# audexdev/Lossless-Audio-Codec

Hardware: AMD Instinct MI355X
Metric: encode Msamples/s at 1/2/4/8 MI355X; byte-identical .lac vs CPU ref (higher is better)
Workload: dtype int64

## Files before the change

### lossless-audio-codec_amd/csrc/api_core.cpp

```cpp
#include "encoder_impl.h"

namespace lacx_host {

Knobs read_knobs() {
    Knobs k;
    auto set = [](const char* name) {
        const char* v = std::getenv(name);
        return v != nullptr;
    };
    auto num = [](const char* name) -> unsigned long long {
        const char* v = std::getenv(name);
        return v ? std::strtoull(v, nullptr, 0) : 0ull;
    };
    k.stream_priority = !set("LACX_NO_STREAM_PRIORITY");
    if (const char* v = std::getenv("LACX_FUSED_EMIT")) k.fused_emit = *v != '0';
    k.direct_packer = set("LACX_DIRECT_PACKER");
    k.packer = !set("LACX_NO_PACKER");
    k.persistent = !set("LACX_NO_PERSISTENT");
    k.debug_drain = set("LACX_DEBUG_DRAIN");
    k.two_copy_streams = !set("LACX_ONE_COPY_STREAM");
    if (const char* v = std::getenv("LACX_STREAM_PRIO")) {
        int a = 0, b = 0, c = 0;
        if (std::sscanf(v, "%d,%d,%d", &a, &b, &c) == 3) {
            k.prio_main = a;
            k.prio_chunks = b;
            k.prio_pack = c;
        }
    }
    k.front_halves = !set("LACX_NO_FRONT_HALVES");
    k.tune.fold_front = !set("LACX_NO_FRONT_FOLD");
    k.lazy_repair = !set("LACX_NO_LAZY_REPAIR");
    k.silent_template = !set("LACX_NO_SILENT_TEMPLATE");
    k.pinned_cap_bytes = num("LACX_PINNED_CAP_BYTES");
    k.debug_skip = (uint32_t)num("LACX_DEBUG_SKIP");
    k.pipe_chunks = (uint32_t)num("LACX_PIPE_CHUNKS");
    if (const char* v = std::getenv("LACX_PIPE_SPLIT")) k.pipe_split = v;
    k.drain_fence = (uint32_t)num("LACX_DRAIN_FENCE");
    if (const char* v = std::getenv("LACX_FANOUT_EXCHANGE")) k.fanout_exchange = std::strcmp(v, "host") == 0 ? 1u : (std::strcmp(v, "rccl") == 0 ? 2u : 0u);
    k.tune.persistent_grid = (uint32_t)num("LACX_PERSISTENT_GRID");
    k.tune.pack_nap = (int)num("LACX_PACK_NAP");
    k.tune.pack_grid = (int)num("LACX_PACK_GRID");
    k.tune.no_pairs = set("LACX_NO_PAIRS");
    return k;
}

double ms_since(clk::time_point t0) { return std::chrono::duration<double, std::milli>(clk::now() - t0).count(); }

int fail(lacx_encoder* e, int code, const std::string& msg) {
    if (e) e->err = msg;
    return code;
}

int hip_fail(lacx_encoder* e, hipError_t err, const char* what) {
    return fail(e, LACX_E_DEVICE, std::string(what) + ": " + hipGetErrorString(err));
}

void big_copy(uint8_t* dst, const uint8_t* src, uint64_t n) {
    constexpr uint64_t kPiece = 4ull << 20;
    const unsigned hw = std::thread::hardware_concurrency();
    const uint64_t want = std::min<uint64_t>(std::min<uint64_t>(8, hw ? hw : 1), n / kPiece);
    if (want < 2) {
        std::memcpy(dst, src, n);
        return;
    }
    std::vector<std::thread> pool;
    const uint64_t per = (n / want + 4095) & ~4095ull;
    for (uint64_t t = 1; t < want; ++t) {
        const uint64_t o = t * per;
        if (o >= n) break;
        pool.emplace_back([=] { std::memcpy(dst + o, src + o, std::min(per, n - o)); });
    }
    std::memcpy(dst, src, std::min(per, n));
    for (auto& th : pool) th.join();
}

int ensure_device(lacx_encoder* e) {
    if (e->device_ready) return LACX_OK;
    int count = 0;
    const hipError_t ce = hipGetDeviceCount(&count);
    if (ce != hipSuccess || count <= 0)
        return fail(e, LACX_E_DEVICE, "no HIP device available: the LAC analysis path has no CPU fallback");
    int dev = e->cfg.device;
    if (dev < 0) HIP_TRY(e, hipGetDevice(&dev), "hipGetDevice");
    if (dev >= count) return fail(e, LACX_E_DEVICE, "HIP device ordinal out of range");
    HIP_TRY(e, hipSetDevice(dev), "hipSetDevice");
    e->device = dev;
    int least = 0, greatest = 0;
    (void)hipDeviceGetStreamPriorityRange(&least, &greatest);
    const bool prio = e->knobs.stream_priority && greatest < least;
    const int normal = (greatest + least) / 2 > greatest ? (greatest + least) / 2 : std::min(greatest + 1, least);
    auto level = [&](int code) { return code < 0 ? greatest : (code == 0 ? normal : least); };
    int i = 0;
    for (auto& s : e->stream) {
        if (prio) {
            const int p = level(i == 0 ? e->knobs.prio_main : (i == kStreams - 1 ? 0 : e->knobs.prio_chunks));
            HIP_TRY(e, hipStreamCreateWithPriority(&s, hipStreamNonBlocking, p), "hipStreamCreate");
        } else {
            HIP_TRY(e, hipStreamCreateWithFlags(&s, hipStreamNonBlocking), "hipStreamCreate");
        }
        ++i;
    }
    for (auto& row : e->ev)
        for (auto& ev : row) HIP_TRY(e, hipEventCreate(&ev), "hipEventCreate");
    for (auto& ev : e->done) HIP_TRY(e, hipEventCreateWithFlags(&ev, hipEventDisableTiming), "hipEventCreate");
    for (auto& ev : e->copied) HIP_TRY(e, hipEventCreateWithFlags(&ev, hipEventDisableTiming), "hipEventCreate");
    HIP_TRY(e, hipEventCreateWithFlags(&e->prologue, hipEventDisableTiming), "hipEventCreate");
    for (auto& ev : e->aux_ev) HIP_TRY(e, hipEventCreateWithFlags(&ev, hipEventDisableTiming), "hipEventCreate");
    HIP_TRY(e, hipHostMalloc((void**)&e->h_totals, sizeof(unsigned long long) * kMaxChunks, 0), "hipHostMalloc");
    HIP_TRY(e, hipHostMalloc((void**)&e->h_err, sizeof(uint32_t) * (kMaxChunks + 8), 0), "hipHostMalloc");
    HIP_TRY(e, hipStreamCreateWithPriority(&e->pack_stream, hipStreamNonBlocking, level(e->knobs.prio_pack)), "hipStreamCreate");
    HIP_TRY(e, hipEventCreateWithFlags(&e->pack_done, hipEventDisableTiming), "hipEventCreate");
    HIP_TRY(e, hipStreamCreateWithFlags(&e->copy_stream, hipStreamNonBlocking), "hipStreamCreate");
    HIP_TRY(e, hipStreamCreateWithFlags(&e->copy_stream2, hipStreamNonBlocking), "hipStreamCreate");
    HIP_TRY(e, hipHostMalloc((void**)&e->h_tspan, sizeof(unsigned long long) * 2 * kMaxChunks, 0), "hipHostMalloc");
    e->device_ready = true;
    return LACX_OK;
}

EmitPool& pool_of(lacx_encoder* e) {
    if (!e->pool) {
        unsigned nt = e->cfg.emit_threads ? e->cfg.emit_threads : std::thread::hardware_concurrency();
        if (nt == 0) nt = 1;
        e->pool.reset(new EmitPool(nt > 1 ? nt - 1 : 0));
    }
    return *e->pool;
}

void free_workspace(lacx_encoder* e) {
    if (e->ws.plans) (void)hipFree(e->ws.plans);
    if (e->ws.bplans) (void)hipFree(e->ws.bplans);
    if (e->ws.need_probe) (void)hipFree(e->ws.need_probe);
    if (e->ws.need_full) (void)hipFree(e->ws.need_full);
    if (e->ws.acorr) (void)hipFree(e->ws.acorr);
    if (e->ws.lpcs) (void)hipFree(e->ws.lpcs);
    if (e->ws.sums) (void)hipFree(e->ws.sums);
    if (e->ws.badidx) (void)hipFree(e->ws.badidx);
    if (e->ws.front_ctr) (void)hipFree(e->ws.front_ctr);
    if (e->ws.block_off) (void)hipFree(e->ws.block_off);
    if (e->ws.table) (void)hipFree(e->ws.table);
    if (e->ws.stream_pre) (void)hipFree(e->ws.stream_pre);
    if (e->zero_region) (void)hipFree(e->zero_region);
    e->zero_region = nullptr;
    e->d_tspan = nullptr;
    e->d_work_ctr = nullptr;
    e->d_silent = nullptr;
    e->ws = DeviceWorkspace{};
    e->ws_blocks = 0;
}

int ensure_workspace(lacx_encoder* e, uint32_t nblocks) {
    if (nblocks > e->ws_blocks) {
        free_workspace(e);
        const size_t slots = (size_t)nblocks * kSlotsPerBlock;
        HIP_TRY(e, hipMalloc((void**)&e->ws.plans, slots * sizeof(ChannelPlan)), "hipMalloc(plans)");
        HIP_TRY(e, hipMalloc((void**)&e->ws.bplans, (size_t)nblocks * sizeof(BlockPlan)), "hipMalloc(bplans)");
        HIP_TRY(e, hipMalloc((void**)&e->ws.need_probe, (size_t)nblocks * 4), "hipMalloc(need)");
        HIP_TRY(e, hipMalloc((void**)&e->ws.need_full, (size_t)nblocks * 4), "hipMalloc(need)");
        HIP_TRY(e, hipMalloc((void**)&e->ws.acorr, slots * 13 * sizeof(int64_t)), "hipMalloc(acorr)");
        HIP_TRY(e, hipMalloc((void**)&e->ws.lpcs, slots * sizeof(LpcSet)), "hipMalloc(lpcs)");
        HIP_TRY(e, hipMalloc((void**)&e->ws.sums, (size_t)nblocks * 12 * sizeof(unsigned long long)), "hipMalloc(sums)");
        HIP_TRY(e, hipMalloc((void**)&e->ws.badidx, (size_t)nblocks * 2 * sizeof(uint32_t)), "hipMalloc(badidx)");
        HIP_TRY(e, hipMalloc((void**)&e->ws.front_ctr, (size_t)nblocks * 2 * sizeof(uint32_t)), "hipMalloc(front counters)");
        HIP_TRY(e, hipMemset(e->ws.front_ctr, 0, (size_t)nblocks * 2 * sizeof(uint32_t)), "hipMemset(front counters)");
        HIP_TRY(e, hipStreamSynchronize(nullptr), "hipStreamSynchronize");
        HIP_TRY(e, hipMalloc((void**)&e->ws.block_off, ((size_t)nblocks + kMaxChunks + 1) * sizeof(unsigned long long)),
                "hipMalloc(block_off)");
        HIP_TRY(e, hipMalloc((void**)&e->ws.table, (size_t)nblocks * 2 * sizeof(uint32_t)), "hipMalloc(table)");
        HIP_TRY(e, hipMalloc((void**)&e->ws.stream_pre, ((size_t)nblocks + 1) * sizeof(unsigned long long)), "hipMalloc(stream prefixes)");

        {
            const size_t items = (size_t)nblocks * 2 + 4;
            const size_t ranges = items / kPackerRangeItems + 2;
            const size_t bytes = items * (2 * sizeof(unsigned long long) + 2 * sizeof(uint32_t)) +
                                 sizeof(unsigned long long) * 2 * kMaxChunks + sizeof(uint32_t) * (kMaxChunks + 8) +
                                 ranges * (sizeof(unsigned long long) + sizeof(uint32_t)) + 16 +
                                 sizeof(uint32_t) * 8 * (kMaxChunks + 1) +
                                 16 + sizeof(SilentTemplate);
            e->zero_bytes = (bytes + 15) & ~(size_t)15;
            HIP_TRY(e, hipMalloc((void**)&e->zero_region, e->zero_bytes), "hipMalloc(zeroed region)");
            uint8_t* p = e->zero_region;
            e->ws.size_rec = reinterpret_cast<unsigned long long*>(p);
            p += items * sizeof(unsigned long long);
            e->ws.ready_rec = reinterpret_cast<unsigned long long*>(p);
            p += items * sizeof(unsigned long long);
            e->d_tspan = reinterpret_cast<unsigned long long*>(p);
            p += sizeof(unsigned long long) * 2 * kMaxChunks;
            e->ws.emitted = reinterpret_cast<uint32_t*>(p);
            p += items * sizeof(uint32_t);
            e->ws.packed = reinterpret_cast<uint32_t*>(p);
            p += items * sizeof(uint32_t);
            e->ws.err_flag = reinterpret_cast<uint32_t*>(p);
            p += sizeof(uint32_t) * (kMaxChunks + 8);
            p = reinterpret_cast<uint8_t*>((reinterpret_cast<uintptr_t>(p) + 7) & ~(uintptr_t)7);
            e->d_range_end = reinterpret_cast<unsigned long long*>(p);
            p += ranges * sizeof(unsigned long long);
            e->d_range_cnt = reinterpret_cast<uint32_t*>(p);
            p += ranges * sizeof(uint32_t);
            p = reinterpret_cast<uint8_t*>((reinterpret_cast<uintptr_t>(p) + 3) & ~(uintptr_t)3);
            e->d_work_ctr = reinterpret_cast<uint32_t*>(p);
            p += sizeof(uint32_t) * 8 * (kMaxChunks + 1);
            p = reinterpret_cast<uint8_t*>((reinterpret_cast<uintptr_t>(p) + 15) & ~(uintptr_t)15);
            e->d_silent = reinterpret_cast<SilentTemplate*>(p);
        }
        e->ws_blocks = nblocks;
    }
    if (nblocks > e->h_blocks) {
        if (e->h_plans) (void)hipHostFree(e->h_plans);
        if (e->h_bplans) (void)hipHostFree(e->h_bplans);
        e->h_plans = nullptr;
        e->h_bplans = nullptr;
        e->h_blocks = 0;
        HIP_TRY(e, hipHostMalloc((void**)&e->h_plans, (size_t)nblocks * kSlotsPerBlock * sizeof(ChannelPlan), 0),
                "hipHostMalloc(plans)");
        HIP_TRY(e, hipHostMalloc((void**)&e->h_bplans, (size_t)nblocks * sizeof(BlockPlan), 0),
                "hipHostMalloc(bplans)");
        e->h_blocks = nblocks;
    }
    return LACX_OK;
}

int ensure_slots(lacx_encoder* e, uint32_t nblocks, int channels, int bit_depth) {
    const unsigned long long stride = (unsigned long long)kMaxBlock * ((bit_depth ? bit_depth : e->cfg.bit_depth) == 16 ? 3u : 5u);
    const unsigned long long need = stride * nblocks * (unsigned)channels + 64u;
    if (const int rc = grow(e, e->slot_mem, need)) return rc;
    e->ws.slots = e->slot_mem.as<uint8_t>();
    e->ws.slot_stride = stride;
    return LACX_OK;
}

int grow(lacx_encoder* e, Buf& b, uint64_t need) {
    const DevErr d = buf_grow(b, need, 0);
    return d ? hip_fail(e, d.e, d.what) : LACX_OK;
}

int ensure_pcm(lacx_encoder* e, uint64_t frames, bool) { return grow(e, e->pcm, frames); }

int validate_stream_args(lacx_encoder* e, const void* left, uint64_t frames) {
    if (left == nullptr || frames == 0) return fail(e, LACX_E_INVALID, "left channel must not be empty");
    if (!rate_ok(e->cfg.sample_rate))
        return fail(e, LACX_E_INVALID, "unsupported sample rate: " + std::to_string(e->cfg.sample_rate));
    if (!(e->cfg.bit_depth == 16 || e->cfg.bit_depth == 24))
        return fail(e, LACX_E_INVALID, "unsupported bit depth: " + std::to_string((int)e->cfg.bit_depth));
    if (e->cfg.stereo_mode > 2)
        return fail(e, LACX_E_INVALID, "unsupported stereo mode: " + std::to_string((int)e->cfg.stereo_mode));
    return LACX_OK;
}

AnalyzeParams make_params(const lacx_encoder* e, uint64_t frames, int channels, int stereo_mode, int bit_depth, int layout) {
    return make_params(param_base(e), frames, channels, stereo_mode, bit_depth, layout);
}

LaunchSet one_stream_set(const AnalyzeParams& prm, const int32_t* left, const int32_t* right, uint32_t fuse_items,
                         uint64_t out_cap) {
    StreamDesc sd{};
    sd.prm = prm;
    sd.left = left;
    sd.right = right;
    sd.first_block = 0;
    sd.first_wg = 0;
    sd.fuse_items = fuse_items;
    sd.out_base = 0;
    sd.out_cap = out_cap;
    return single_set(sd);
}
const LaunchSet& bind(LaunchSet& ls) {
    if (ls.br.table == nullptr) ls.streams = &ls.br.single;
    return ls;
}

DeviceWorkspace ws_at(const DeviceWorkspace& ws, uint32_t first_block) {
    DeviceWorkspace w = ws;
    const size_t s = (size_t)first_block * kSlotsPerBlock;
    w.plans += s;
    w.bplans += first_block;
    w.need_probe += first_block;
    w.need_full += first_block;
    w.acorr += s * 13;
    w.lpcs += s;
    w.sums += (size_t)first_block * 12;
    w.badidx += (size_t)first_block * 2;
    if (w.front_ctr) w.front_ctr += (size_t)first_block * 2;
    w.table += (size_t)first_block * 2;
    return w;
}

void add_chunk_timing(lacx_encoder* e, int c) {
    float f = 0;
    if (hipEventElapsedTime(&f, e->ev[c][0], e->ev[c][4]) == hipSuccess) e->timing.analysis_ms += f;
    if (hipEventElapsedTime(&f, e->ev[c][0], e->ev[c][1]) == hipSuccess) e->timing.ingest_ms += f;
    if (hipEventElapsedTime(&f, e->ev[c][1], e->ev[c][2]) == hipSuccess) e->timing.probe_ms += f;
    if (hipEventElapsedTime(&f, e->ev[c][2], e->ev[c][3]) == hipSuccess) e->timing.full_ms += f;
    (void)hipGetLastError();
}

void count_slots(lacx_encoder* e, uint32_t first, uint32_t count) {
    uint64_t fs = 0, ps = 0;
    for (uint32_t b = first; b < first + count; ++b) {
        const ChannelPlan* s = e->h_plans + (size_t)b * kSlotsPerBlock;
        for (int i = 0; i < 4; ++i) fs += s[i].valid;
        for (int i = 4; i < kSlotsPerBlock; ++i) ps += s[i].valid;
    }
    e->timing.full_slots += fs;
    e->timing.probe_slots += ps;
}

int check_sample_range(lacx_encoder* e, uint32_t nb) {
    e->bad_channel = -1;
    for (int pass = 0; pass < 2; ++pass) {
        for (uint32_t b = 0; b < nb; ++b) {
            const BlockPlan& bp = e->h_bplans[b];
            if (!bp.invalid) continue;
            const bool is_right = (bp.first_bad >> 31) != 0;
            if ((pass == 0) == is_right) continue;
            const uint64_t idx = (uint64_t)b * kMaxBlock + (bp.first_bad & 0x7FFFFFFFu);
            e->bad_channel = is_right ? 1 : 0;
            e->bad_index = idx;
            return fail(e, LACX_E_INVALID,
                        std::string(is_right ? "right" : "left") + " sample at index " + std::to_string(idx) +
                            " is outside the configured PCM bit depth");
        }
    }
    return LACX_OK;
}

void reset_device_timing(lacx_encoder* e) {
    e->timing.analysis_ms = e->timing.ingest_ms = e->timing.probe_ms = e->timing.full_ms = 0;
    e->timing.full_slots = e->timing.probe_slots = 0;
    e->timing.full_launches = 0;
}

StreamParams stream_params(const lacx_config& c, int channels) {
    StreamParams sp;
    sp.sample_rate = c.sample_rate;
    sp.bit_depth = c.bit_depth;
    sp.channels = (uint8_t)channels;
    sp.stereo_mode = channels == 2 ? c.stereo_mode : 0;
    return sp;
// ... 146 lines not shown
```

### lossless-audio-codec_amd/csrc/k_front.hip

```cpp
#include <hip/hip_runtime.h>

#include "kernels_internal.h"
#include "x87.h"

namespace lacx {

__device__ __forceinline__ uint64_t zz64(int64_t v) {
    return v >= 0 ? ((uint64_t)v << 1) : ((((uint64_t)(-(v + 1))) << 1) | 1u);
}

__device__ __forceinline__ uint64_t approx_rice_bits(uint64_t sum, uint64_t count) {
    if (count == 0) return 0;
    const uint64_t mean = (sum + (count >> 1)) / count;
    uint32_t k = mean <= 1u ? 0u : 64u - (uint32_t)__clzll((long long)(mean - 1u));
    k = k > 31u ? 31u : k;
    return (sum >> k) + count * (uint64_t)(k + 1u);
}

constexpr int kIngestTile = 4096;
static_assert(kIngestThreads == kProbe, "one probe sample per thread");

__device__ __forceinline__ bool slot_channel_used(const AnalyzeParams& prm, int ch) {
    if (prm.channels == 1) return ch == 0;
    if (prm.stereo_mode == 0) return ch < 2;
    if (prm.stereo_mode == 1) return ch >= 2;
    return true;
}

__device__ __forceinline__ void reduce13(const int64_t* acc, unsigned long long* s_ac, int64_t* out, int tid) {
    if (tid < 13) s_ac[tid] = 0;
    __syncthreads();
#pragma unroll
    for (int k = 0; k < 13; ++k) {
        const uint64_t t = wave_sum_u64((uint64_t)acc[k]);
        if ((tid & 63) == 0) atomicAdd(&s_ac[k], (unsigned long long)t);
    }
    __syncthreads();
    if (tid < 13) out[tid] = (int64_t)s_ac[tid];
    __syncthreads();
}

__device__ __forceinline__ void stereo_block(const AnalyzeParams& prm, uint32_t blk, uint32_t nb, bool live, int tid,
                                             const unsigned long long* __restrict__ sums, const uint32_t* __restrict__ badidx,
                                             BlockPlan* __restrict__ bplans, uint32_t* __restrict__ need_probe,
                                             uint32_t* __restrict__ need_full);

__device__ __forceinline__ void ingest_done(uint32_t* __restrict__ front_ctr, unsigned int* s_last, const AnalyzeParams& prm,
                                            uint32_t blk, uint32_t nb, const unsigned long long* __restrict__ sums,
                                            const uint32_t* __restrict__ badidx, BlockPlan* __restrict__ bplans,
                                            uint32_t* __restrict__ need_probe, uint32_t* __restrict__ need_full) {
    if (!front_ctr) return;
    const int tid = threadIdx.x;
    if (tid == 0) {
        asm volatile("s_waitcnt vmcnt(0)" ::: "memory");
        *s_last = atomicAdd(&front_ctr[(size_t)blk * 2], 1u) == 3u ? 1u : 0u;
    }
    __syncthreads();
    if (*s_last == 0u || tid >= 64) return;
    if (tid == 0) front_ctr[(size_t)blk * 2] = 0u;
    stereo_block(prm, blk, nb, tid < 16, tid, sums, badidx, bplans, need_probe, need_full);
}

__global__ __launch_bounds__(kIngestThreads, 5) void k_ingest(BatchRef br, unsigned long long* __restrict__ sums,
                                                           uint32_t* __restrict__ badidx,
                                                           int64_t* __restrict__ acorr, uint32_t* __restrict__ front_ctr,
                                                           BlockPlan* __restrict__ bplans, uint32_t* __restrict__ need_probe,
                                                           uint32_t* __restrict__ need_full) {
    __shared__ int4 s_plane[4][kIngestThreads + 1];
    __shared__ __align__(16) int32_t s_win[3][12 + kProbe];
    __shared__ unsigned long long s_ac[13];
    __shared__ unsigned long long s_sum[3];
    __shared__ unsigned int s_bad;
    uint32_t blk, chsel;
    xcd_slot(blockIdx.x, 4u, gridDim.x >> 2, blk, chsel);
    const StreamDesc sd = stream_of_block_uniform(br, blk);
    const AnalyzeParams prm = sd.prm;
    const int32_t* __restrict__ L = sd.left;
    const int32_t* __restrict__ R = sd.right;
    const uint32_t lblk = blk - sd.first_block;
    const int ch = (int)chsel;
    const bool used = slot_channel_used(prm, ch);
    const bool container_bounds = prm.layout == PCM_INTERLEAVED_I16 || (prm.layout == PCM_INTERLEAVED_I24 && prm.bit_depth == 24);
    const bool validate = ch < 2 && ch < prm.channels && prm.bit_depth != 0 && !container_bounds;
    const uint32_t nb = block_frames(prm, lblk);
    if (!used && !validate) {
        if (ch < 2 && threadIdx.x == 0) agent_store(&badidx[blk * 2 + ch], 0xFFFFFFFFu);
        ingest_done(front_ctr, &s_bad, prm, blk, nb, sums, badidx, bplans, need_probe, need_full);
        return;
    }
    const int tid = threadIdx.x, lane = tid & 63;
    const int64_t bstart = (int64_t)lblk * kMaxBlock;
    const SlotSrc src = slot_src(prm, L, R, ch);
    const bool est = prm.channels == 2 && prm.stereo_mode == 2;
    const int32_t lo = prm.bit_depth == 16 ? -32768 : -0x800000;
    const int32_t hi = prm.bit_depth == 16 ? 32767 : 0x7FFFFF;
    if (tid < 3) s_sum[tid] = 0;
    if (tid == 0) s_bad = 0xFFFFFFFFu;
    if (tid < 4) s_plane[tid][0] = make_int4(0, 0, 0, 0);
    __syncthreads();

    constexpr int kPerThread = kIngestTile / kIngestThreads;
    static_assert(kPerThread == 16, "four 4-sample groups per thread and tile");
    int64_t acc[13];
#pragma unroll
    for (int k = 0; k < 13; ++k) acc[k] = 0;
    uint64_t sraw = 0, sdif = 0, sant = 0;
    uint32_t bad = 0xFFFFFFFFu;
    for (uint32_t base = 0; base < nb; base += kIngestTile) {
        const uint32_t first = base + 16u * (uint32_t)tid;
        const int rem = (int)nb - (int)first;
        const int cnt = rem < 0 ? 0 : (rem > 16 ? 16 : rem);
        int32_t w[28];
        load_chunk<16>(src, bstart + first, cnt, bstart + (int64_t)nb - 1, w + 12);
#pragma unroll
        for (int i = 0; i < 16; ++i) {
            if (i >= cnt) w[12 + i] = 0;
            else if (validate && (w[12 + i] < lo || w[12 + i] > hi)) bad = bad < first + (uint32_t)i ? bad : first + (uint32_t)i;
        }
#pragma unroll
        for (int c = 0; c < 4; ++c)
            s_plane[c][tid + 1] = make_int4(w[12 + 4 * c], w[13 + 4 * c], w[14 + 4 * c], w[15 + 4 * c]);
        __syncthreads();
        int4 carry = make_int4(0, 0, 0, 0);
        if (tid >= 1 && tid <= 3) carry = s_plane[tid][kIngestThreads];
#pragma unroll
        for (int c = 1; c < 4; ++c) {
            const int4 h = s_plane[c][tid];
            w[4 * (c - 1)] = h.x;
            w[4 * (c - 1) + 1] = h.y;
            w[4 * (c - 1) + 2] = h.z;
            w[4 * (c - 1) + 3] = h.w;
        }
        if (used) {
#pragma unroll
            for (int i = 0; i < 16; ++i) {
#pragma unroll
                for (int k = 0; k < 13; ++k) acc[k] += (int64_t)w[12 + i] * (int64_t)w[12 + i - k];
            }
            if (est) {
                auto zz32 = [](int32_t v) { return ((uint32_t)v << 1) ^ (uint32_t)(v >> 31); };
                uint32_t traw = 0, tdif = 0, tant = 0;
#pragma unroll
                for (int i = 0; i < 16; ++i) {
                    if (i < cnt) {
                        const int32_t x0 = w[12 + i], prev = w[11 + i];
                        const uint32_t raw = zz32(x0);
                        const bool head = (first + (uint32_t)i) == 0u;
                        traw += raw;
                        tdif += head ? raw : zz32((int32_t)((uint32_t)x0 - (uint32_t)prev));
                        tant += head ? raw : zz32((int32_t)((uint32_t)x0 + (uint32_t)prev));
                    }
                }
                sraw += traw;
                sdif += tdif;
                sant += tant;
            }
        }
        __syncthreads();
        if (tid >= 1 && tid <= 3) s_plane[tid][0] = carry;
    }
    if (used) reduce13(acc, s_ac, acorr + ((size_t)blk * kSlotsPerBlock + ch) * 13, tid);

    if (est && nb > (uint32_t)kFullCompareLimit) {
        if (tid < 36) s_win[tid / 12][tid % 12] = 0;
        for (int w = 1; w <= 3; ++w) {
            const SlotGeom g = slot_geom(prm, lblk, w * 4 + ch);
            s_win[w - 1][12 + tid] = slot_fetch(src, g.start + tid);
        }
        __syncthreads();
        const int wv = tid >> 6;
        if (wv < 3) {
            int32_t v[16];
#pragma unroll
            for (int c = 0; c < 4; ++c) {
                const int4 q = *reinterpret_cast<const int4*>(&s_win[wv][4 * lane + 4 * c]);
                v[4 * c] = q.x;
                v[4 * c + 1] = q.y;
                v[4 * c + 2] = q.z;
                v[4 * c + 3] = q.w;
            }
            int64_t* out = acorr + ((size_t)blk * kSlotsPerBlock + (wv + 1) * 4 + ch) * 13;
#pragma unroll
            for (int k = 0; k < 13; ++k) {
                int64_t a = 0;
#pragma unroll
                for (int i = 0; i < 4; ++i) a += (int64_t)v[12 + i] * (int64_t)v[12 + i - k];
                const uint64_t t = wave_sum_u64((uint64_t)a);
                if (lane == 0) out[k] = (int64_t)t;
            }
        }
    }

    if (est) {
        const uint64_t t0 = wave_sum_u64(sraw), t1 = wave_sum_u64(sdif), t2 = wave_sum_u64(sant);
        if (lane == 0) {
            atomicAdd(&s_sum[0], (unsigned long long)t0);
            atomicAdd(&s_sum[1], (unsigned long long)t1);
            atomicAdd(&s_sum[2], (unsigned long long)t2);
        }
    }
    if (bad != 0xFFFFFFFFu) atomicMin(&s_bad, bad);
    __syncthreads();
    if (tid == 0) {
        if (est) {
            agent_store(&sums[(size_t)blk * 12 + ch], s_sum[0]);
            agent_store(&sums[(size_t)blk * 12 + 4 + ch], s_sum[1]);
            agent_store(&sums[(size_t)blk * 12 + 8 + ch], s_sum[2]);
        }
        if (validate || ch < 2) agent_store(&badidx[blk * 2 + ch], s_bad);
    }
    __syncthreads();
    ingest_done(front_ctr, &s_bad, prm, blk, nb, sums, badidx, bplans, need_probe, need_full);
}

constexpr int kStereoLanes = 16;
__device__ __forceinline__ void stereo_block(const AnalyzeParams& prm, uint32_t blk, uint32_t nb, bool live, int tid,
                                             const unsigned long long* __restrict__ sums, const uint32_t* __restrict__ badidx,
                                             BlockPlan* __restrict__ bplans, uint32_t* __restrict__ need_probe,
                                             uint32_t* __restrict__ need_full) {
    const int sub = tid & (kStereoLanes - 1), grp = tid & ~(kStereoLanes - 1);
    const bool stereo = prm.channels == 2;
    const bool est = stereo && prm.stereo_mode == 2;
    uint64_t bits = 0;
    if (est && live && sub < 12) bits = approx_rice_bits(agent_load(&sums[(size_t)blk * 12 + sub]), nb);
    auto from = [&](int lane_in_group) {
        const uint32_t lo = (uint32_t)__shfl((int)(uint32_t)bits, grp + lane_in_group, 64);
        const uint32_t hi = (uint32_t)__shfl((int)(uint32_t)(bits >> 32), grp + lane_in_group, 64);
        return ((uint64_t)hi << 32) | lo;
    };
    uint64_t chbits[4];
    bool active = false;
#pragma unroll
    for (int c = 0; c < 4; ++c) {
        const uint64_t raw = from(c), dif = from(4 + c), ant = from(8 + c);
        uint64_t mn = raw < dif ? raw : dif;
        if (ant < mn) mn = ant;
        chbits[c] = mn;
        active = active || (raw < dif) || (ant < dif);
    }
    if (!live || sub != 0) return;
    BlockPlan bp;
    bp.choose_ms = 0;
    bp.uncertain = 0;
    bp.est_ms = 0;
    const uint32_t badl = agent_load(&badidx[blk * 2]), badr = stereo ? agent_load(&badidx[blk * 2 + 1]) : 0xFFFFFFFFu;
    bp.invalid = (badl != 0xFFFFFFFFu) || (badr != 0xFFFFFFFFu);
    bp.first_bad = (badl != 0xFFFFFFFFu) ? badl : (badr != 0xFFFFFFFFu ? (badr | 0x80000000u) : 0xFFFFFFFFu);
    bp.frames = nb;
    bp.pad = 0;
    uint32_t nprobe = 0, nfull = 0;
    if (!stereo) {
        nfull = 1u;
    } else if (prm.stereo_mode == 0) {
        nfull = 0x3u;
    } else if (prm.stereo_mode == 1) {
        nfull = 0xCu;
        bp.choose_ms = 1;
    } else {
        const uint64_t lr = chbits[0] + chbits[1], ms = chbits[2] + chbits[3];
        const uint64_t smaller = lr < ms ? lr : ms;
        const uint64_t diff = lr >= ms ? lr - ms : ms - lr;
        bp.est_ms = ms < lr;
        bp.choose_ms = bp.est_ms;
        bp.uncertain = smaller == 0 || diff == 0 || active || diff <= smaller / 100u;
        if (!bp.uncertain) {
            nfull = bp.est_ms ? 0xCu : 0x3u;
        } else if (nb <= (uint32_t)kFullCompareLimit) {
            nfull = 0xFu;
        } else if (agent_load(&sums[(size_t)blk * 12]) == 0ull && agent_load(&sums[(size_t)blk * 12 + 1]) == 0ull) {
            nfull = 0x3u;
            bp.choose_ms = 0;
        } else {
            nprobe = 0xFFF0u;
        }
    }
    bplans[blk] = bp;
    need_probe[blk] = nprobe;
    need_full[blk] = nfull;
}

__global__ __launch_bounds__(64) void k_stereo(BatchRef br, const unsigned long long* __restrict__ sums,
                                               const uint32_t* __restrict__ badidx, BlockPlan* __restrict__ bplans,
                                               uint32_t* __restrict__ need_probe, uint32_t* __restrict__ need_full) {
    const int tid = threadIdx.x;
    const uint32_t blk = blockIdx.x * (64 / kStereoLanes) + (uint32_t)(tid / kStereoLanes);
    const bool live = blk < br.total_blocks;
    const StreamDesc sd = stream_of_block(br, live ? blk : 0u);
    const uint32_t nb = live ? block_frames(sd.prm, blk - sd.first_block) : 0u;
    stereo_block(sd.prm, blk, nb, live, tid, sums, badidx, bplans, need_probe, need_full);
}


__global__ __launch_bounds__(kLevThreads) void k_levinson(BatchRef br, const int64_t* __restrict__ acorr,
                                                          const uint32_t* __restrict__ need_probe,
                                                          LpcSet* __restrict__ lpcs) {
    extern __shared__ __align__(16) unsigned char lev_raw[];
    LevMem& lm = *reinterpret_cast<LevMem*>(lev_raw);
    const uint32_t id = blockIdx.x * kLevThreads + threadIdx.x;
    const uint32_t nblk = br.total_blocks;
    const int slot = (int)(id / nblk);
    const uint32_t blk = id % nblk;
    if (slot >= kSlotsPerBlock) return;
    const StreamDesc sd = stream_of_block(br, blk);
    const AnalyzeParams prm = sd.prm;
    const SlotGeom g = slot_geom(prm, blk - sd.first_block, slot);
    if (!g.defined) return;
    if (prm.channels == 2 && slot < 4) {
        if (prm.stereo_mode == 0 && (slot & 3) >= 2) return;
        if (prm.stereo_mode == 1 && (slot & 3) < 2) return;
    }
    if (slot >= 4 && !((need_probe[blk] >> slot) & 1u)) return;
    const uint32_t gid = blk * kSlotsPerBlock + (uint32_t)slot;
    const int mvo = (g.n > 1) ? (int)((g.n - 1 < 32u) ? g.n - 1 : 32u) : 0;
    struct LdsArray {
        uint64_t (*m)[kLevThreads];
        uint32_t (*es)[kLevThreads];
        int lane;
        __device__ xf80 get(int i) const {
            const uint32_t w = es[i][lane];
            return xf80{m[i][lane], (int32_t)(w & 0x7FFFFFFFu) - (1 << 21), w >> 31};
        }
        __device__ void set(int i, xf80 x) {
            m[i][lane] = x.m;
            es[i][lane] = (x.s << 31) | ((uint32_t)(x.e + (1 << 21)) & 0x7FFFFFFFu);
        }
    };
    const int lane = (int)threadIdx.x;
    LdsArray Rv{lm.m[0], lm.es[0], lane}, av{lm.m[1], lm.es[1], lane}, pv{lm.m[2], lm.es[2], lane};
    const int64_t* r = acorr + (size_t)gid * 13;
    LpcSet* out = &lpcs[gid];
    levinson_candidates_t([r](int i) { return r[i]; }, mvo, Rv, av, pv,
                          [out](int ci, int j, int16_t v) { out->coef[ci][j] = v; },
                          [out](int ci, uint8_t v) { out->used[ci] = v; });
    out->pad = 0;
}

__global__ __launch_bounds__(64) void k_decide(BatchRef br, int phase, BlockPlan* __restrict__ bplans,
                                               const uint32_t* __restrict__ need_probe,
                                               uint32_t* __restrict__ need_full,
                                               const ChannelPlan* __restrict__ plans) {
    const int tid = threadIdx.x, sub = tid & 15;
    const uint32_t blk = blockIdx.x * 4u + (uint32_t)(tid >> 4);
    if (br.table == nullptr && (br.single.prm.channels != 2 || br.single.prm.stereo_mode != 2)) return;
    const bool live = blk < br.total_blocks;
    BlockPlan bp{};
    if (live) bp = bplans[blk];
    const bool mine = live && bp.uncertain &&
                      (phase == 1 ? need_probe[blk] != 0 : bp.frames <= (uint32_t)kFullCompareLimit);
    const bool take = mine && (phase == 1 ? sub >= 4 : sub < 4);
    const uint32_t bytes = take ? plans[(size_t)blk * kSlotsPerBlock + sub].payload_bytes : 0u;
    const bool is_ms = (sub & 3) >= 2;
    uint32_t lr = is_ms ? 0u : bytes, ms = is_ms ? bytes : 0u;
#pragma unroll
    for (int d = 1; d < 16; d <<= 1) {
        lr += (uint32_t)__shfl_xor((int)lr, d, 64);
        ms += (uint32_t)__shfl_xor((int)ms, d, 64);
    }
    if (!mine || sub != 0) return;
    bp.choose_ms = ms < lr;
    bplans[blk] = bp;
    if (phase == 1) need_full[blk] = bp.choose_ms ? 0xCu : 0x3u;
}

hipError_t set_kernel_attrs_front() {
    return hipFuncSetAttribute(reinterpret_cast<const void*>(&k_levinson), hipFuncAttributeMaxDynamicSharedMemorySize,
                               (int)sizeof(LevMem));
}

}
```

### lossless-audio-codec_amd/csrc/lacx_types.h

```cpp
#pragma once
#include <stddef.h>
#include <stdint.h>

struct lacx_block_info;
struct lacx_run_detector;
struct lacx_run;
struct lacx_loudness_row;
struct lacx_truepeak_row;
struct lacx_spectrum_row;

namespace lacx {

constexpr int kMaxBlock = 16384;
constexpr int kMaxParts = 256;
constexpr int kMinPartition = 32;
constexpr int kMaxPartitionOrder = 8;
constexpr size_t kDecodeTailPad = 128;
constexpr int kProbe = 256;
constexpr int kFullCompareLimit = 4096;

enum : int { CH_L = 0, CH_R = 1, CH_M = 2, CH_S = 3 };

constexpr int kSlotsPerBlock = 16;

struct LpcSet {
    int16_t coef[5][13];
    uint8_t used[5];
    uint8_t pad;
};

struct ChannelPlan {
    uint8_t predictor_type;
    uint8_t order;
    uint8_t partition_order;
    uint8_t valid;
    int16_t coef[12];
    uint32_t payload_bytes;
    uint64_t total_bits;
    uint8_t part_mode_k[kMaxParts];
};

struct BlockPlan {
    uint8_t choose_ms;
    uint8_t uncertain;
    uint8_t est_ms;
    uint8_t invalid;
    uint32_t frames;
    uint32_t first_bad;
    uint32_t pad;
};

struct AnalyzeParams {
    uint64_t frames;
    uint32_t num_blocks;
    uint32_t first_block;
    int32_t channels;
    int32_t stereo_mode;
    int32_t bit_depth;
    int32_t zero_run;
    int32_t partitioning;
    uint32_t debug_skip;
    int32_t layout;
    uint32_t stream_base;
};

struct StreamDesc {
    AnalyzeParams prm;
    const int32_t* left;
    const int32_t* right;
    uint32_t first_block;
    uint32_t first_wg;
    uint32_t fuse_items;
    uint32_t pad;
    unsigned long long out_base;
    unsigned long long out_cap;
};

struct BatchRef {
    const StreamDesc* table;
    uint32_t nstreams;
    uint32_t total_blocks;
    StreamDesc single;
};

struct VerifySource {
    const void* data0;
    const void* data1;
    uint32_t layout;
    uint32_t pad;
};
struct VerifyWords {
    unsigned long long count;
    unsigned long long key;
    int32_t decoded, source;
    uint32_t block;
    uint32_t pad;
};

struct DigestWords {
    uint32_t raw;
    uint32_t pad;
};
struct DigestSource {
    const void* data0;
    const void* data1;
    unsigned long long frames;
    uint32_t layout;
    uint8_t channels, bit_depth, pad[2];
};
constexpr unsigned long long kDigestClean = ~0ull;
struct DigestPcmArgs {
    uint32_t nitems = 0;
    unsigned long long total_units = 0;
    const unsigned long long* unit_off = nullptr;
    const DigestSource* src = nullptr;
    DigestWords* res = nullptr;
    unsigned long long* bad = nullptr;
};

struct DecodeItem {
    int32_t* left;
    int32_t* right;
    uint8_t* wav;
    unsigned long long frame0;
    unsigned long long frames;
    unsigned long long pay_off;
    uint32_t block0, blocks;
    uint32_t pay_bits;
    uint8_t channels, stereo_mode, bit_depth, version;
};
struct WindowOut {
    void* left;
    void* right;
    unsigned long long start;
    unsigned long long frames;
};
struct DecodeArgs {
    uint32_t nitems = 0, total_blocks = 0;
    const DecodeItem* items = nullptr;
    const uint32_t* blk_item = nullptr;
    uint32_t lanes = 0;
    const uint32_t* lane_blk = nullptr;
    uint32_t nv2 = 0;
    const uint32_t* v2_items = nullptr;
    const uint8_t* payload = nullptr;
    const unsigned long long* byte_off = nullptr;
    const unsigned long long* frame_off = nullptr;
    uint32_t* status = nullptr;
    uint8_t* ms_flag = nullptr;
    bool wav = false;
    const unsigned long long* unit_off = nullptr;
    unsigned long long total_units = 0;
    const WindowOut* window = nullptr;
    bool f32 = false;
    const VerifySource* verify = nullptr;
    VerifyWords* verify_res = nullptr;
    DigestWords* digest = nullptr;
    const uint32_t* present = nullptr;
    uint32_t* block_raw = nullptr;
    const uint32_t* block_expect = nullptr;
    const uint32_t* judged = nullptr;
    bool no_output = false;
};
struct BlockPcmArgs {
    DigestPcmArgs pcm;
    uint32_t grid = 0;
    const unsigned long long* block_off = nullptr;
    uint32_t* raw = nullptr;
};
struct StatsAcc;
struct StatsArgs {
    DecodeArgs dec;
    StatsAcc* rows = nullptr;
};
struct StatsPcmArgs {
    DigestPcmArgs pcm;
    uint32_t grid = 0;
    const unsigned long long* block_off = nullptr;
    StatsAcc* rows = nullptr;
};
struct RunsItem;
struct RunsList;
struct RunsRow;
struct RunsArgs {
    DecodeArgs dec;
    uint32_t nitems = 0;
    unsigned long long total_tiles = 0;
    const unsigned long long* tile_off = nullptr;
    const RunsItem* items = nullptr;
    const lacx_run_detector* dets = nullptr;
    RunsList* lists = nullptr;
    RunsRow* rows = nullptr;
    lacx_run* runs = nullptr;
    const DigestSource* src = nullptr;
    unsigned long long* bad = nullptr;
};
constexpr uint32_t kInspectPartSlots = 256;
static_assert(kInspectPartSlots == (uint32_t)kMaxParts, "a channel block has at most kMaxParts partitions");
struct InspectArgs {
    DecodeArgs dec;
    lacx_block_info* rows = nullptr;
    uint8_t* mode_k = nullptr;
    uint32_t* part_bits = nullptr;
};
constexpr uint32_t kLoudChunk = 256;
struct LoudFilter {
    double sb[3], sna[2];
    double hb[3], hna[2];
    double A[4][4];
};
struct LoudState {
    double s[4];
};
struct LoudPartial {
    double p[2];
};
struct LoudItem {
    const void* data0;
    const void* data1;
    unsigned long long frames;
    unsigned long long used;
    unsigned long long lane0;
    unsigned long long row0;
    uint32_t chunks, rows;
    uint32_t sub, layout;
    uint8_t channels, bit_depth, rate, validate;
    uint32_t pad;
};
struct LoudArgs {
    uint32_t nitems = 0;
    unsigned long long total_chunks = 0, total_rows = 0;
    const LoudFilter* filters = nullptr;
    const LoudItem* items = nullptr;
    const unsigned long long* chunk_off = nullptr;
    const unsigned long long* row_off = nullptr;
    LoudState* states = nullptr;
    LoudPartial* partials = nullptr;
    lacx_loudness_row* rows = nullptr;
    unsigned long long* bad = nullptr;
};
constexpr uint32_t kTpTileFrames = 1024;
constexpr uint32_t kTpThreads = 256;
constexpr uint32_t kTpTaps = 12, kTpPhases = 4;
constexpr uint32_t kTpFlush = kTpTaps - 1;
constexpr uint32_t kTpHistory = 12;
constexpr uint32_t kTpRowFrames = 16384;
constexpr uint32_t kTpPosBits = 18;
struct TpAcc {
    unsigned long long key[2];
    uint32_t sample_peak[2];
    uint32_t pad[2];
};
struct TpItem {
    const void* data0;
    const void* data1;
    unsigned long long frames;
    unsigned long long row0;
    uint32_t tiles, rows;
    uint32_t layout;
    uint8_t channels, bit_depth, validate, pad;
};
struct TpArgs {
    uint32_t nitems = 0;
    unsigned long long total_tiles = 0, total_rows = 0;
    const TpItem* items = nullptr;
    const unsigned long long* tile_off = nullptr;
    TpAcc* rows = nullptr;
    unsigned long long* bad = nullptr;
};
constexpr uint32_t kSpThreads = 256;
constexpr uint32_t kSpBands = 64;
constexpr uint32_t kSpRowFrames = 16384;
constexpr uint32_t kSpMinLog = 8, kSpMaxLog = 12;
struct SpItem {
    const void* data0;
    const void* data1;
    unsigned long long frames;
    unsigned long long row0;
    unsigned long long windows;
    uint32_t rows;
    uint32_t layout;
    uint8_t channels, bit_depth, validate, pad[5];
};
struct SpArgs {
    uint32_t nitems = 0;
    uint32_t logn = 0;
    unsigned long long total_rows = 0;
    const SpItem* items = nullptr;
    const unsigned long long* row_off = nullptr;
    const double* window = nullptr;
    const double* twiddle = nullptr;
    lacx_spectrum_row* rows = nullptr;
    unsigned long long* bad = nullptr;
};
}
```

Before: 24760.

## Compute ingest autocorrelation with int8 MFMA on split byte planes

Replaces the per-thread int64 VALU autocorrelation loop in k_ingest with int8 MFMA (16x16x64) products. Samples are split into signed byte planes (3 for 16-bit, 4 for 24-bit) and the 13 lags are recombined from the shifted plane products. It also lowers launch bounds occupancy from 5 to 3 workgroups and enlarges the LDS staging buffer. The VALU path stays reachable through a debug bit set by LACX_INGEST_MFMA=0. The risks are exactness of the plane recombination, extra LDS traffic, and lower occupancy.

Result: slower. 24430 (-1.3%).

```diff
diff --git a/lossless-audio-codec_amd/csrc/api_core.cpp b/lossless-audio-codec_amd/csrc/api_core.cpp
--- a/lossless-audio-codec_amd/csrc/api_core.cpp
+++ b/lossless-audio-codec_amd/csrc/api_core.cpp
@@ -33,6 +33,9 @@
     k.silent_template = !set("LACX_NO_SILENT_TEMPLATE");
     k.pinned_cap_bytes = num("LACX_PINNED_CAP_BYTES");
     k.debug_skip = (uint32_t)num("LACX_DEBUG_SKIP");
+    if (const char* v = std::getenv("LACX_INGEST_MFMA")) {
+        if (*v == '0') k.debug_skip |= lacx::kIngestValuBit;
+    }
     k.pipe_chunks = (uint32_t)num("LACX_PIPE_CHUNKS");
     if (const char* v = std::getenv("LACX_PIPE_SPLIT")) k.pipe_split = v;
     k.drain_fence = (uint32_t)num("LACX_DRAIN_FENCE");
diff --git a/lossless-audio-codec_amd/csrc/k_front.hip b/lossless-audio-codec_amd/csrc/k_front.hip
--- a/lossless-audio-codec_amd/csrc/k_front.hip
+++ b/lossless-audio-codec_amd/csrc/k_front.hip
@@ -18,6 +18,9 @@
 }
 
 constexpr int kIngestTile = 4096;
+#ifndef LACX_INGEST_WGS
+#define LACX_INGEST_WGS 3
+#endif
 static_assert(kIngestThreads == kProbe, "one probe sample per thread");
 
 __device__ __forceinline__ bool slot_channel_used(const AnalyzeParams& prm, int ch) {
@@ -61,12 +64,231 @@
     stereo_block(prm, blk, nb, tid < 16, tid, sums, badidx, bplans, need_probe, need_full);
 }
 
-__global__ __launch_bounds__(kIngestThreads, 5) void k_ingest(BatchRef br, unsigned long long* __restrict__ sums,
+struct IngestBlock {
+    SlotSrc src;
+    int64_t bstart;
+    uint32_t nb;
+    int32_t lo, hi;
+    bool validate, used, est;
+    uint64_t sraw, sdif, sant;
+    uint32_t bad;
+};
+
+__device__ __forceinline__ void ingest_check16(IngestBlock& ib, uint32_t first, int cnt, int32_t* x) {
+#pragma unroll
+    for (int i = 0; i < 16; ++i) {
+        if (i >= cnt) x[i] = 0;
+        else if (ib.validate && (x[i] < ib.lo || x[i] > ib.hi)) ib.bad = ib.bad < first + (uint32_t)i ? ib.bad : first + (uint32_t)i;
+    }
+}
+
+__device__ __forceinline__ int ingest_fetch16(IngestBlock& ib, uint32_t first, int32_t* x) {
+    const int rem = (int)ib.nb - (int)first;
+    const int cnt = rem < 0 ? 0 : (rem > 16 ? 16 : rem);
+    load_chunk<16>(ib.src, ib.bstart + first, cnt, ib.bstart + (int64_t)ib.nb - 1, x);
+    ingest_check16(ib, first, cnt, x);
+    return cnt;
+}
+
+__device__ __forceinline__ void ingest_proxy16(IngestBlock& ib, uint32_t first, int cnt, const int32_t* x) {
+    auto zz32 = [](int32_t v) { return ((uint32_t)v << 1) ^ (uint32_t)(v >> 31); };
+    uint32_t traw = 0, tdif = 0, tant = 0;
+#pragma unroll
+    for (int i = 0; i < 16; ++i) {
+        if (i < cnt) {
+            const int32_t x0 = x[i], prev = x[i - 1];
+            const uint32_t raw = zz32(x0);
+            const bool head = (first + (uint32_t)i) == 0u;
+            traw += raw;
+            tdif += head ? raw : zz32((int32_t)((uint32_t)x0 - (uint32_t)prev));
+            tant += head ? raw : zz32((int32_t)((uint32_t)x0 + (uint32_t)prev));
+        }
+    }
+    ib.sraw += traw;
+    ib.sdif += tdif;
+    ib.sant += tant;
+}
+
+__device__ __forceinline__ void ingest_valu(IngestBlock& ib, int4 (*s_plane)[kIngestThreads + 1], unsigned long long* s_ac,
+                                         int64_t* out) {
+    const int tid = threadIdx.x;
+    if (tid < 4) s_plane[tid][0] = make_int4(0, 0, 0, 0);
+    __syncthreads();
+    static_assert(kIngestTile / kIngestThreads == 16, "four 4-sample groups per thread and tile");
+    int64_t acc[13];
+#pragma unroll
+    for (int k = 0; k < 13; ++k) acc[k] = 0;
+    for (uint32_t base = 0; base < ib.nb; base += kIngestTile) {
+        const uint32_t first = base + 16u * (uint32_t)tid;
+        int32_t w[28];
+        const int cnt = ingest_fetch16(ib, first, w + 12);
+#pragma unroll
+        for (int c = 0; c < 4; ++c)
+            s_plane[c][tid + 1] = make_int4(w[12 + 4 * c], w[13 + 4 * c], w[14 + 4 * c], w[15 + 4 * c]);
+        __syncthreads();
+        int4 carry = make_int4(0, 0, 0, 0);
+        if (tid >= 1 && tid <= 3) carry = s_plane[tid][kIngestThreads];
+#pragma unroll
+        for (int c = 1; c < 4; ++c) {
+            const int4 h = s_plane[c][tid];
+            w[4 * (c - 1)] = h.x;
+            w[4 * (c - 1) + 1] = h.y;
+            w[4 * (c - 1) + 2] = h.z;
+            w[4 * (c - 1) + 3] = h.w;
+        }
+        if (ib.used) {
+#pragma unroll
+            for (int i = 0; i < 16; ++i) {
+#pragma unroll
+                for (int k = 0; k < 13; ++k) acc[k] += (int64_t)w[12 + i] * (int64_t)w[12 + i - k];
+            }
+            if (ib.est) ingest_proxy16(ib, first, cnt, w + 12);
+        }
+        __syncthreads();
+        if (tid >= 1 && tid <= 3) s_plane[tid][0] = carry;
+    }
+    if (ib.used) reduce13(acc, s_ac, out, tid);
+}
+
+template <int ND>
+struct IngestMfma {
+    typedef int v4i __attribute__((ext_vector_type(4)));
+    static constexpr int kPass = 2 * kIngestTile;
+    static constexpr int kRow = 16 + 2 * kIngestThreads;
+    static constexpr int kStageBytes = ND * 16 * kRow;
+    static constexpr int kSums = 2 * ND - 1;
+    static_assert(kMaxBlock == 2 * kPass && kIngestTile == 16 * kIngestThreads, "two passes of two columns per thread");
+    struct Acc {
+        v4i p[kSums], m[kSums];
+    };
+
+    __device__ static __forceinline__ void stage(const int32_t* x0, const int32_t* x1, unsigned char* s_stage, bool first_pass) {
+        const int tid = threadIdx.x;
+#pragma unroll
+        for (int c = 0; c < 16; ++c) {
+            const uint32_t y0 = ((uint32_t)x0[1 + c] + 0x80808080u) ^ 0x80808080u, y1 = ((uint32_t)x1[1 + c] + 0x80808080u) ^ 0x80808080u;
+            const uint32_t u01 = __builtin_amdgcn_perm(y1, y0, 0x05010400u), u23 = __builtin_amdgcn_perm(y1, y0, 0x07030602u);
+#pragma unroll
+            for (int s = 0; s < ND; ++s) {
+                const uint32_t d = ((s < 2 ? u01 : u23) >> (16 * (s & 1))) & 0xFFFFu;
+                unsigned char* row = s_stage + (s * 16 + c) * kRow;
+                if (tid == kIngestThreads - 1) {
+                    const uint32_t before = first_pass ? 0u : row[16 + 2 * kIngestThreads - 1];
+                    *reinterpret_cast<uint16_t*>(row + 14) = (uint16_t)(before | ((d & 0xFFu) << 8));
+                }
+                *reinterpret_cast<uint16_t*>(row + 16 + 2 * tid) = (uint16_t)d;
+            }
+        }
+    }
+
+    __device__ static __forceinline__ void multiply(const unsigned char* s_stage, Acc& acc) {
+        const int tid = threadIdx.x, lane = tid & 63, wv = tid >> 6;
+        const int r = lane & 15, q = lane >> 4, arow = (16 - r) & 15;
+#pragma unroll
+        for (int step = wv; step < 2 * kIngestThreads / 64; step += kIngestThreads / 64) {
+            const int off = 16 + (step * 4 + q) * 16;
+            v4i b[ND], am[ND], ap[ND];
+#pragma unroll
+            for (int s = 0; s < ND; ++s) {
+                b[s] = *reinterpret_cast<const v4i*>(s_stage + (s * 16 + r) * kRow + off);
+                const v4i f = *reinterpret_cast<const v4i*>(s_stage + (s * 16 + arow) * kRow + off);
+                const int pv = *reinterpret_cast<const int*>(s_stage + (s * 16 + arow) * kRow + off - 4);
+                const v4i sh = v4i{(int)__builtin_amdgcn_alignbyte((uint32_t)f[0], (uint32_t)pv, 2u),
+                                   (int)__builtin_amdgcn_alignbyte((uint32_t)f[1], (uint32_t)f[0], 2u),
+                                   (int)__builtin_amdgcn_alignbyte((uint32_t)f[2], (uint32_t)f[1], 2u),
+                                   (int)__builtin_amdgcn_alignbyte((uint32_t)f[3], (uint32_t)f[2], 2u)};
+                const v4i zero = v4i{0, 0, 0, 0};
+                am[s] = r == 0 ? zero : f;
+                ap[s] = r == 0 ? f : (r <= 12 ? sh : zero);
+            }
+#pragma unroll
+            for (int s = 0; s < ND; ++s) {
+#pragma unroll
+                for (int t = 0; t < ND; ++t) {
+                    acc.p[s + t] = __builtin_amdgcn_mfma_i32_16x16x64_i8(ap[s], b[t], acc.p[s + t], 0, 0, 0);
+                    acc.m[s + t] = __builtin_amdgcn_mfma_i32_16x16x64_i8(am[s], b[t], acc.m[s + t], 0, 0, 0);
+                }
+            }
+        }
+    }
+
+    __device__ static __forceinline__ void finish(const Acc& acc, unsigned long long* s_ac) {
+        const int lane = threadIdx.x & 63, r = lane & 15, q = lane >> 4;
+#pragma unroll
+        for (int i = 0; i < 4; ++i) {
+            uint64_t vp = 0, vm = 0;
+#pragma unroll
+            for (int g = 0; g < kSums; ++g) {
+                vp += (uint64_t)(int64_t)acc.p[g][i] << (8 * g);
+                vm += (uint64_t)(int64_t)acc.m[g][i] << (8 * g);
+            }
+            const int lp = 4 * q + i + r, lm = lp - 16;
+            if (lp <= 12) atomicAdd(&s_ac[lp], (unsigned long long)vp);
+            if (lm >= 0 && lm <= 12) atomicAdd(&s_ac[lm], (unsigned long long)vm);
+        }
+    }
+
+    __device__ static __forceinline__ void run(IngestBlock& ib, unsigned char* s_stage, int32_t (*s_edge)[4],
+                                               unsigned long long* s_ac, int64_t* out) {
+        const int tid = threadIdx.x, lane = tid & 63, wv = tid >> 6;
+        constexpr int kWaves = kIngestThreads / 64;
+        Acc acc;
+#pragma unroll
+        for (int i = 0; i < kSums; ++i) acc.p[i] = acc.m[i] = v4i{0, 0, 0, 0};
+        if (tid < 13) s_ac[tid] = 0;
+#pragma unroll 1
+        for (int p = 0; p < 2; ++p) {
+            const uint32_t base = (uint32_t)(p * kPass);
+            if (base >= ib.nb) break;
+            const uint32_t first0 = base + 16u * (uint32_t)tid, first1 = first0 + (uint32_t)kIngestTile;
+            int32_t x0[17], x1[17];
+            int cnt0 = 16, cnt1 = 16;
+            if (ib.nb - base >= (uint32_t)kPass &&
+                wave_all(span_ok<16>(ib.src, ib.bstart + first0) && span_ok<16>(ib.src, ib.bstart + first1))) {
+                stage_span<16>(ib.src, ib.bstart + first0, x0 + 1);
+                stage_span<16>(ib.src, ib.bstart + first1, x1 + 1);
+                ingest_check16(ib, first0, 16, x0 + 1);
+                ingest_check16(ib, first1, 16, x1 + 1);
+            } else {
+                cnt0 = ingest_fetch16(ib, first0, x0 + 1);
+                cnt1 = ingest_fetch16(ib, first1, x1 + 1);
+            }
+            if (!ib.used) continue;
+            if (lane == 63) {
+                s_edge[wv][2 * p] = x0[16];
+                s_edge[wv][2 * p + 1] = x1[16];
+            }
+            stage(x0, x1, s_stage, p == 0);
+            __syncthreads();
+            multiply(s_stage, acc);
+            if (ib.est) {
+                auto proxy = [&](int m, uint32_t first, int cnt, int32_t* x) {
+                    int32_t before = __shfl_up(x[16], 1, 64);
+                    if (lane == 0) before = wv > 0 ? s_edge[wv - 1][m] : s_edge[kWaves - 1][m > 0 ? m - 1 : 0];
+                    x[0] = before;
+                    ingest_proxy16(ib, first, cnt, x + 1);
+                };
+                proxy(2 * p, first0, cnt0, x0);
+                proxy(2 * p + 1, first1, cnt1, x1);
+            }
+            __syncthreads();
+        }
+        if (!ib.used) return;
+        finish(acc, s_ac);
+        __syncthreads();
+        if (tid < 13) out[tid] = (int64_t)s_ac[tid];
+        __syncthreads();
+    }
+};
+
+__global__ __launch_bounds__(kIngestThreads, LACX_INGEST_WGS) void k_ingest(BatchRef br, unsigned long long* __restrict__ sums,
                                                            uint32_t* __restrict__ badidx,
                                                            int64_t* __restrict__ acorr, uint32_t* __restrict__ front_ctr,
                                                            BlockPlan* __restrict__ bplans, uint32_t* __restrict__ need_probe,
                                                            uint32_t* __restrict__ need_full) {
-    __shared__ int4 s_plane[4][kIngestThreads + 1];
+    __shared__ __align__(16) unsigned char s_stage[IngestMfma<4>::kStageBytes];
+    static_assert(sizeof(s_stage) >= sizeof(int4) * 4 * (kIngestThreads + 1), "the vector form's planes fit");
+    __shared__ int32_t s_edge[kIngestThreads / 64][4];
     __shared__ __align__(16) int32_t s_win[3][12 + kProbe];
     __shared__ unsigned long long s_ac[13];
     __shared__ unsigned long long s_sum[3];
@@ -96,70 +318,14 @@
     const int32_t hi = prm.bit_depth == 16 ? 32767 : 0x7FFFFF;
     if (tid < 3) s_sum[tid] = 0;
     if (tid == 0) s_bad = 0xFFFFFFFFu;
-    if (tid < 4) s_plane[tid][0] = make_int4(0, 0, 0, 0);
-    __syncthreads();
-
-    constexpr int kPerThread = kIngestTile / kIngestThreads;
-    static_assert(kPerThread == 16, "four 4-sample groups per thread and tile");
-    int64_t acc[13];
-#pragma unroll
-    for (int k = 0; k < 13; ++k) acc[k] = 0;
-    uint64_t sraw = 0, sdif = 0, sant = 0;
-    uint32_t bad = 0xFFFFFFFFu;
-    for (uint32_t base = 0; base < nb; base += kIngestTile) {
-        const uint32_t first = base + 16u * (uint32_t)tid;
-        const int rem = (int)nb - (int)first;
-        const int cnt = rem < 0 ? 0 : (rem > 16 ? 16 : rem);
-        int32_t w[28];
-        load_chunk<16>(src, bstart + first, cnt, bstart + (int64_t)nb - 1, w + 12);
-#pragma unroll
-        for (int i = 0; i < 16; ++i) {
-            if (i >= cnt) w[12 + i] = 0;
-            else if (validate && (w[12 + i] < lo || w[12 + i] > hi)) bad = bad < first + (uint32_t)i ? bad : first + (uint32_t)i;
-        }
-#pragma unroll
-        for (int c = 0; c < 4; ++c)
-            s_plane[c][tid + 1] = make_int4(w[12 + 4 * c], w[13 + 4 * c], w[14 + 4 * c], w[15 + 4 * c]);
-        __syncthreads();
-        int4 carry = make_int4(0, 0, 0, 0);
-        if (tid >= 1 && tid <= 3) carry = s_plane[tid][kIngestThreads];
-#pragma unroll
-        for (int c = 1; c < 4; ++c) {
-            const int4 h = s_plane[c][tid];
-            w[4 * (c - 1)] = h.x;
-            w[4 * (c - 1) + 1] = h.y;
-            w[4 * (c - 1) + 2] = h.z;
-            w[4 * (c - 1) + 3] = h.w;
-        }
-        if (used) {
-#pragma unroll
-            for (int i = 0; i < 16; ++i) {
-#pragma unroll
-                for (int k = 0; k < 13; ++k) acc[k] += (int64_t)w[12 + i] * (int64_t)w[12 + i - k];
-            }
-            if (est) {
-                auto zz32 = [](int32_t v) { return ((uint32_t)v << 1) ^ (uint32_t)(v >> 31); };
-                uint32_t traw = 0, tdif = 0, tant = 0;
-#pragma unroll
-                for (int i = 0; i < 16; ++i) {
-                    if (i < cnt) {
-                        const int32_t x0 = w[12 + i], prev = w[11 + i];
-                        const uint32_t raw = zz32(x0);
-                        const bool head = (first + (uint32_t)i) == 0u;
-                        traw += raw;
-                        tdif += head ? raw : zz32((int32_t)((uint32_t)x0 - (uint32_t)prev));
-                        tant += head ? raw : zz32((int32_t)((uint32_t)x0 + (uint32_t)prev));
-                    }
-                }
-                sraw += traw;
-                sdif += tdif;
-                sant += tant;
-            }
-        }
-        __syncthreads();
-        if (tid >= 1 && tid <= 3) s_plane[tid][0] = carry;
-    }
-    if (used) reduce13(acc, s_ac, acorr + ((size_t)blk * kSlotsPerBlock + ch) * 13, tid);
+    __syncthreads();
+    IngestBlock ib{src, bstart, nb, lo, hi, validate, used, est, 0, 0, 0, 0xFFFFFFFFu};
+    int64_t* const ac_out = acorr + ((size_t)blk * kSlotsPerBlock + ch) * 13;
+    if (prm.debug_skip & kIngestValuBit) ingest_valu(ib, reinterpret_cast<int4(*)[kIngestThreads + 1]>(s_stage), s_ac, ac_out);
+    else if (prm.bit_depth == 16) IngestMfma<3>::run(ib, s_stage, s_edge, s_ac, ac_out);
+    else IngestMfma<4>::run(ib, s_stage, s_edge, s_ac, ac_out);
+    const uint64_t sraw = ib.sraw, sdif = ib.sdif, sant = ib.sant;
+    const uint32_t bad = ib.bad;
 
     if (est && nb > (uint32_t)kFullCompareLimit) {
         if (tid < 36) s_win[tid / 12][tid % 12] = 0;
diff --git a/lossless-audio-codec_amd/csrc/lacx_types.h b/lossless-audio-codec_amd/csrc/lacx_types.h
--- a/lossless-audio-codec_amd/csrc/lacx_types.h
+++ b/lossless-audio-codec_amd/csrc/lacx_types.h
@@ -49,6 +49,8 @@
     uint32_t first_bad;
     uint32_t pad;
 };
+
+constexpr uint32_t kIngestValuBit = 1u << 31;
 
 struct AnalyzeParams {
     uint64_t frames;
```
